# aligirayhanozbay/poisson_CNN

Measured on AMD Instinct MI355X. Metric: grids/sec (fwd+bwd) at 1024^2, higher is better.
Workload: dtype f32; 1 GPU; c4: Homogeneous_Poisson_NN_Legacy(hpnn.json) full train step (fwd+bwd+loss+Adam), 8 x 1024x1024 Dirichlet grids per GPU; global_batch=8, parallelism=dp1, math=fp32, ranks_seen=1

## Files before the change

poisson_cnn_amd/csrc/conv_small.hip:

```cpp
#include "pcnn_internal.h"
#include "conv_epilogue.h"

int pcnn_conv_small_fwd(pcnn_handle h, const pcnn_conv_desc* d, const float* x, const float* w, const float* bias, const float* bn_scale,
                        const float* bn_shift, const float* residual, float* y, float* act_out);
int pcnn_conv_small_wgrad(pcnn_handle h, const pcnn_conv_desc* d, const float* x, const float* dz, float* dw, void* workspace, size_t workspace_bytes);
bool pcnn_conv_fwd_takes_narrow_route(pcnn_handle h, const pcnn_conv_desc* d);
bool pcnn_conv_small_fwd_eligible(const pcnn_conv_desc* d);
bool pcnn_conv_small_wgrad_eligible(const pcnn_conv_desc* d);
size_t pcnn_conv_small_wgrad_workspace(const pcnn_conv_desc* d);

namespace {

constexpr int STH = 8, STW = 32;
__host__ __device__ constexpr int lds_stride(int CI) { return CI == 16 ? 20 : CI; }

struct SmallParams {
  const float* x; const float* wp; const float* bias; const float* bn_scale; const float* bn_shift; const float* res; float* y; float* act_out;
  unsigned* absmax;
  int N, H, W, Cin, ldx, Ho, Wo, Cout, ldy, pt, pl, pad_mode; float pad_value; int act; float alpha;
  int ld_res, ld_act, tiles_x, tiles_y, vec_in, vec_out;
  const float* gact = nullptr; float* y2 = nullptr; float* bpart = nullptr;
  int ld_gact = 0, ld_y2 = 0, gmode = 0; float galpha = 1.f;
};

__device__ __forceinline__ int pad_index_sel(int i, int n, int mode) {
  const int refl = mode == PCNN_PAD_SYMMETRIC ? (i < 0 ? -i - 1 : 2 * n - 1 - i) : (i < 0 ? -i : 2 * n - 2 - i);
  const int rc = min(max(refl, 0), n - 1);
  return (unsigned)i < (unsigned)n ? i : (mode == PCNN_PAD_CONSTANT ? -1 : rc);
}

template <int K, int CI, int CIS = lds_stride(CI)>
__device__ __forceinline__ void stage_tile(float* __restrict__ lds, const float* __restrict__ xin, int H, int W, int Cin, int ldx, int y0, int x0, int pt, int pl,
                                           int pad_mode, float pad_value, int vec) {
  constexpr int TR = STH + K - 1, TC = STW + K - 1, Q = CI / 4;
  for (int u = threadIdx.x; u < TR * TC * Q; u += blockDim.x) {
    const int q = u % Q, pix = u / Q, r = pix / TC, c = pix - r * TC;
    const int sy = pcnn_pad_index(y0 + r - pt, H, pad_mode), sx = pcnn_pad_index(x0 + c - pl, W, pad_mode);
    f32x4 v;
    if (sy < 0 || sx < 0) {
      v = (f32x4){pad_value, pad_value, pad_value, pad_value};
    } else {
      const float* src = xin + ((int64_t)sy * W + sx) * ldx + 4 * q;
      if (vec && 4 * q + 3 < Cin) v = *reinterpret_cast<const f32x4*>(src);
      else {
#pragma unroll
        for (int j = 0; j < 4; ++j) v[j] = 4 * q + j < Cin ? src[j] : 0.f;
      }
    }
#pragma unroll
    for (int j = 0; j < 4; ++j)
      if (4 * q + j >= Cin) v[j] = 0.f;
    *reinterpret_cast<f32x4*>(lds + pix * CIS + 4 * q) = v;
  }
}

template <int K, int CI, int CIS = lds_stride(CI)>
__device__ __forceinline__ void stage_tile_batched(float* __restrict__ lds, const float* __restrict__ xin, int H, int W, int ldx, int y0, int x0, int pt, int pl,
                                                   int pad_mode, float pad_value) {
  constexpr int TR = STH + K - 1, TC = STW + K - 1, Q = CI / 4, TOTAL = TR * TC * Q, NX = (TOTAL + 255) / 256;
  f32x4 v[NX];
  unsigned okm = 0;
#pragma unroll
  for (int i = 0; i < NX; ++i) {
    const int u = threadIdx.x + i * 256, q = u % Q, pix = u / Q, r = pix / TC, c = pix - r * TC;
    const int sy = pad_index_sel(y0 + r - pt, H, pad_mode), sx = pad_index_sel(x0 + c - pl, W, pad_mode);
    const bool ok = u < TOTAL && sy >= 0 && sx >= 0;
    const int64_t idx = ok ? ((int64_t)sy * W + sx) * ldx + 4 * q : 0;
    v[i] = *reinterpret_cast<const f32x4*>(xin + idx);
    okm |= ok ? (1u << i) : 0u;
  }
  const f32x4 padv = {pad_value, pad_value, pad_value, pad_value};
#pragma unroll
  for (int i = 0; i < NX; ++i) {
    const int u = threadIdx.x + i * 256;
    if (u < TOTAL) *reinterpret_cast<f32x4*>(lds + (u / Q) * CIS + 4 * (u % Q)) = ((okm >> i) & 1u) ? v[i] : padv;
  }
}

template <int K, int CI, int CO, bool POST = false>
__global__ __launch_bounds__(256, (CI * CO <= 64 ? 8 : 4)) void conv_small_fwd_kernel(SmallParams p) {
  constexpr int TC = STW + K - 1, CIS = lds_stride(CI);
  extern __shared__ __attribute__((aligned(16))) float lds[];
  int tile = blockIdx.x;
  const int tx = tile % p.tiles_x; tile /= p.tiles_x;
  const int ty = tile % p.tiles_y;
  const int n = tile / p.tiles_y;
  const int y0 = ty * STH, x0 = tx * STW;
  if (p.vec_in && (p.Cin & 3) == 0) stage_tile_batched<K, CI>(lds, p.x + (int64_t)n * p.H * p.W * p.ldx, p.H, p.W, p.ldx, y0, x0, p.pt, p.pl, p.pad_mode, p.pad_value);
  else stage_tile<K, CI>(lds, p.x + (int64_t)n * p.H * p.W * p.ldx, p.H, p.W, p.Cin, p.ldx, y0, x0, p.pt, p.pl, p.pad_mode, p.pad_value, p.vec_in);
  __syncthreads();
  const int r = threadIdx.x >> 5, c = threadIdx.x & 31;
  float acc[CO];
#pragma unroll
  for (int o = 0; o < CO; ++o) acc[o] = 0.f;
  const float* wp = p.wp;
#pragma unroll 1
  for (int i = 0; i < K; ++i)
#pragma unroll
    for (int j = 0; j < K; ++j) {
      const float* px = lds + ((r + i) * TC + (c + j)) * CIS;
      float xv[CI];
#pragma unroll
      for (int q = 0; q < CI / 4; ++q) {
        const f32x4 v = *reinterpret_cast<const f32x4*>(px + 4 * q);
        xv[4 * q] = v[0]; xv[4 * q + 1] = v[1]; xv[4 * q + 2] = v[2]; xv[4 * q + 3] = v[3];
      }
#pragma unroll
      for (int ci = 0; ci < CI; ++ci)
#pragma unroll
        for (int o = 0; o < CO; ++o) acc[o] = fmaf(xv[ci], wp[((i * K + j) * CI + ci) * CO + o], acc[o]);
    }
  const int oy = y0 + r, ox = x0 + c;
  float ymax = 0.f;
  if constexpr (POST) {
    float bs[CO];
#pragma unroll
    for (int o = 0; o < CO; ++o) bs[o] = 0.f;
    if (oy < p.Ho && ox < p.Wo) {
      const int64_t pix = ((int64_t)n * p.Ho + oy) * p.Wo + ox;
      f32x4 rr[CO / 4], gg[CO / 4];
#pragma unroll
      for (int q = 0; q < CO / 4; ++q) {
        const int cq = 4 * q < p.Cout ? 4 * q : 0;
        gg[q] = *reinterpret_cast<const f32x4*>(p.gact + pix * p.ld_gact + cq);
        if (p.res) rr[q] = *reinterpret_cast<const f32x4*>(p.res + pix * p.ld_res + cq);
      }
#pragma unroll
      for (int q = 0; q < CO / 4; ++q) {
        if (4 * q < p.Cout) {
          f32x4 v = {acc[4 * q], acc[4 * q + 1], acc[4 * q + 2], acc[4 * q + 3]};
          if (p.res) {
#pragma unroll
            for (int j = 0; j < 4; ++j) v[j] += rr[q][j];
          }
          if (p.y2) *reinterpret_cast<f32x4*>(p.y2 + pix * p.ld_y2 + 4 * q) = v;
#pragma unroll
          for (int j = 0; j < 4; ++j) {
            const float gq = gg[q][j];
            v[j] *= p.gmode == PCNN_ACT_TANH ? 1.f - gq * gq : (gq > 0.f ? 1.f : p.galpha);
            bs[4 * q + j] = v[j];
            ymax = fmaxf(ymax, fabsf(v[j]));
          }
          *reinterpret_cast<f32x4*>(p.y + pix * p.ldy + 4 * q) = v;
        }
      }
    }
    if (p.bpart) {
      __syncthreads();
#pragma unroll
      for (int o = 0; o < CO; ++o) {
        float v = bs[o];
#pragma unroll
        for (int m = 32; m > 0; m >>= 1) v += __shfl_xor(v, m);
        if ((threadIdx.x & 63) == 0) lds[(threadIdx.x >> 6) * CO + o] = v;
      }
      __syncthreads();
      if (threadIdx.x < CO) p.bpart[(int64_t)blockIdx.x * CO + threadIdx.x] = ((lds[threadIdx.x] + lds[CO + threadIdx.x]) + lds[2 * CO + threadIdx.x]) + lds[3 * CO + threadIdx.x];
    }
    conv_epilogue_absmax(p.absmax, ymax);
    return;
  }
  if (oy < p.Ho && ox < p.Wo) {
    const int64_t pix = ((int64_t)n * p.Ho + oy) * p.Wo + ox;
    float out[CO];
#pragma unroll
    for (int o = 0; o < CO; ++o) {
      float v = 0.f;
      if (o < p.Cout) {
        v = pcnn_act(acc[o] + (p.bias ? p.bias[o] : 0.f), p.act, p.alpha);
        if (p.act_out && !p.vec_out) p.act_out[pix * p.ld_act + o] = v;
      }
      out[o] = v;
    }
    if (p.vec_out) {
      f32x4 rr[CO / 4];
      if (p.res) {
#pragma unroll
        for (int q = 0; q < CO / 4; ++q) rr[q] = *reinterpret_cast<const f32x4*>(p.res + pix * p.ld_res + (4 * q < p.Cout ? 4 * q : 0));
      }
      if (p.act_out) {
#pragma unroll
        for (int q = 0; q < CO / 4; ++q)
          if (4 * q < p.Cout) *reinterpret_cast<f32x4*>(p.act_out + pix * p.ld_act + 4 * q) = (f32x4){out[4 * q], out[4 * q + 1], out[4 * q + 2], out[4 * q + 3]};
      }
#pragma unroll
      for (int q = 0; q < CO / 4; ++q) {
        if (4 * q < p.Cout) {
          f32x4 v = {out[4 * q], out[4 * q + 1], out[4 * q + 2], out[4 * q + 3]};
          if (p.bn_scale) {
#pragma unroll
            for (int j = 0; j < 4; ++j) v[j] = v[j] * p.bn_scale[4 * q + j] + p.bn_shift[4 * q + j];
          }
          if (p.res) {
#pragma unroll
            for (int j = 0; j < 4; ++j) v[j] += rr[q][j];
          }
          *reinterpret_cast<f32x4*>(p.y + pix * p.ldy + 4 * q) = v;
#pragma unroll
          for (int j = 0; j < 4; ++j) ymax = fmaxf(ymax, fabsf(v[j]));
        }
      }
    } else {
#pragma unroll
      for (int o = 0; o < CO; ++o) {
        if (o < p.Cout) {
          float v = out[o];
          if (p.bn_scale) v = v * p.bn_scale[o] + p.bn_shift[o];
          if (p.res) v += p.res[pix * p.ld_res + o];
          p.y[pix * p.ldy + o] = v;
          ymax = fmaxf(ymax, fabsf(v));
        }
      }
    }
  }
  conv_epilogue_absmax(p.absmax, ymax);
}

__global__ void pack_small_kernel(const float* __restrict__ w, float* __restrict__ wp, int taps, int Cin, int Cout, int CI, int CO) {
  const int total = taps * CI * CO;
  for (int i = blockIdx.x * blockDim.x + threadIdx.x; i < total; i += gridDim.x * blockDim.x) {
    const int o = i % CO; int r = i / CO; const int ci = r % CI; const int t = r / CI;
    wp[i] = (ci < Cin && o < Cout) ? w[((int64_t)t * Cin + ci) * Cout + o] : 0.f;
  }
}

template <int K, int CI, int CO>
void launch_small_fwd(pcnn_handle h, const SmallParams& p, int64_t nblk) {
  constexpr size_t lds = (size_t)(STH + K - 1) * (STW + K - 1) * lds_stride(CI) * sizeof(float);
  static_assert(lds >= 4 * 16 * sizeof(float), "the POST epilogue reduces 4 waves x CO sums through the tile's LDS");
  if (p.gact) hipLaunchKernelGGL((conv_small_fwd_kernel<K, CI, CO, true>), dim3((unsigned)nblk), dim3(256), lds, h->stream, p);
  else hipLaunchKernelGGL((conv_small_fwd_kernel<K, CI, CO, false>), dim3((unsigned)nblk), dim3(256), lds, h->stream, p);
}

template <int K, int CI>
bool dispatch_co(pcnn_handle h, const SmallParams& p, int64_t nblk, int CO) {
  switch (CO) {
    case 4: launch_small_fwd<K, CI, 4>(h, p, nblk); return true;
    case 8: launch_small_fwd<K, CI, 8>(h, p, nblk); return true;
    case 12: launch_small_fwd<K, CI, 12>(h, p, nblk); return true;
    case 16: launch_small_fwd<K, CI, 16>(h, p, nblk); return true;
  }
  return false;
}
template <int K>
bool dispatch_ci(pcnn_handle h, const SmallParams& p, int64_t nblk, int CI, int CO) {
  switch (CI) {
    case 4: return dispatch_co<K, 4>(h, p, nblk, CO);
    case 8: return dispatch_co<K, 8>(h, p, nblk, CO);
    case 12: return dispatch_co<K, 12>(h, p, nblk, CO);
    case 16: return dispatch_co<K, 16>(h, p, nblk, CO);
  }
  return false;
}

struct SmallWgradParams {
  const float* x; const float* dz; float* part;
  int N, H, W, Cin, ldx, Ho, Wo, Cout, lddz, pt, pl, pad_mode; float pad_value;
  int tiles_x, tiles_y, ntiles, S, vec_in, vec_dz;
};

template <int K, int CI, int CO>
__global__ __launch_bounds__(64 * K) void conv_small_wgrad_kernel(SmallWgradParams p) {
  constexpr int TR = STH + K - 1, TC = STW + K - 1, CIS = CI, COS = CO;
  constexpr int NT = 64 * K, QX = CI / 4, QZ = CO / 4, NX = (TR * TC * QX + NT - 1) / NT, NZ = (STH * STW * QZ + NT - 1) / NT;
  extern __shared__ __attribute__((aligned(16))) float lds[];
  float* xs = lds;
  float* zs = lds + TR * TC * CIS + 16;
  const int tid = threadIdx.x, lane = tid & 63, ch = lane & 15, kk = lane >> 4;
  const int wave = __builtin_amdgcn_readfirstlane(tid >> 6);
  const int split = blockIdx.x;
  constexpr int GP = CI <= 4 ? 4 : (CI <= 8 ? 2 : 1), CPT = 16 / GP, NM = (K + GP - 1) / GP;
  const int js = ch / CPT, cc = ch % CPT;
  f32x4 acc[NM];
#pragma unroll
  for (int g = 0; g < NM; ++g) acc[g] = (f32x4){0.f, 0.f, 0.f, 0.f};
  const bool b_ok = ch < CO;
  f32x4 xr[NX], zr[NZ];
  unsigned xok = ~0u, zok = ~0u;
  const bool fast = p.vec_in && p.vec_dz && (p.Cin & 3) == 0 && (p.Cout & 3) == 0;
  const f32x4 padv = {p.pad_value, p.pad_value, p.pad_value, p.pad_value}, zero4 = {0.f, 0.f, 0.f, 0.f};
  auto fetch = [&](int tile) {
    int tt = tile;
    const int tx = tt % p.tiles_x; tt /= p.tiles_x;
    const int ty = tt % p.tiles_y;
    const int n = tt / p.tiles_y;
    const int y0 = ty * STH, x0 = tx * STW;
    const float* xin = p.x + (int64_t)n * p.H * p.W * p.ldx;
    const float* zin = p.dz + (int64_t)n * p.Ho * p.Wo * p.lddz;
    if (fast) {
#pragma unroll
      for (int i = 0; i < NX; ++i) {
        const int u = tid + i * NT, q = u % QX, pix = u / QX, r = pix / TC, c = pix - r * TC;
        const int sy = pad_index_sel(y0 + r - p.pt, p.H, p.pad_mode), sx = pad_index_sel(x0 + c - p.pl, p.W, p.pad_mode);
        const bool ok = u < TR * TC * QX && sy >= 0 && sx >= 0;
        xr[i] = *reinterpret_cast<const f32x4*>(xin + (ok ? ((int64_t)sy * p.W + sx) * p.ldx + 4 * q : 0));
        xok = ok ? (xok | (1u << i)) : (xok & ~(1u << i));
      }
#pragma unroll
      for (int i = 0; i < NZ; ++i) {
        const int u = tid + i * NT, q = u % QZ, pix = u / QZ, r = pix / STW, c = pix - r * STW;
        const bool ok = u < STH * STW * QZ && y0 + r < p.Ho && x0 + c < p.Wo;
        zr[i] = *reinterpret_cast<const f32x4*>(zin + (ok ? ((int64_t)(y0 + r) * p.Wo + x0 + c) * p.lddz + 4 * q : 0));
        zok = ok ? (zok | (1u << i)) : (zok & ~(1u << i));
      }
      return;
    }
#pragma unroll
    for (int i = 0; i < NX; ++i) {
      const int u = tid + i * NT, q = u % QX, pix = u / QX, r = pix / TC, c = pix - r * TC;
      f32x4 v = {0.f, 0.f, 0.f, 0.f};
      if (u < TR * TC * QX) {
        const int sy = pcnn_pad_index(y0 + r - p.pt, p.H, p.pad_mode), sx = pcnn_pad_index(x0 + c - p.pl, p.W, p.pad_mode);
        if (sy < 0 || sx < 0) v = (f32x4){p.pad_value, p.pad_value, p.pad_value, p.pad_value};
        else {
          const float* src = xin + ((int64_t)sy * p.W + sx) * p.ldx + 4 * q;
          if (p.vec_in && 4 * q + 3 < p.Cin) v = *reinterpret_cast<const f32x4*>(src);
          else {
#pragma unroll
            for (int j = 0; j < 4; ++j) v[j] = 4 * q + j < p.Cin ? src[j] : 0.f;
          }
        }
#pragma unroll
        for (int j = 0; j < 4; ++j)
          if (4 * q + j >= p.Cin) v[j] = 0.f;
      }
      xr[i] = v;
    }
#pragma unroll
    for (int i = 0; i < NZ; ++i) {
      const int u = tid + i * NT, q = u % QZ, pix = u / QZ, r = pix / STW, c = pix - r * STW;
      f32x4 v = {0.f, 0.f, 0.f, 0.f};
      if (u < STH * STW * QZ && y0 + r < p.Ho && x0 + c < p.Wo) {
        const float* src = zin + ((int64_t)(y0 + r) * p.Wo + x0 + c) * p.lddz + 4 * q;
        if (p.vec_dz && 4 * q + 3 < p.Cout) v = *reinterpret_cast<const f32x4*>(src);
        else {
#pragma unroll
          for (int j = 0; j < 4; ++j) v[j] = 4 * q + j < p.Cout ? src[j] : 0.f;
        }
      }
      zr[i] = v;
    }
  };
  int tile = split;
  if (tile < p.ntiles) fetch(tile);
  for (; tile < p.ntiles; tile += p.S) {
    __syncthreads();
#pragma unroll
    for (int i = 0; i < NX; ++i) {
      const int u = tid + i * NT;
      if (u < TR * TC * QX) *reinterpret_cast<f32x4*>(xs + (u / QX) * CIS + 4 * (u % QX)) = ((xok >> i) & 1u) ? xr[i] : padv;
    }
#pragma unroll
    for (int i = 0; i < NZ; ++i) {
      const int u = tid + i * NT;
      if (u < STH * STW * QZ) *reinterpret_cast<f32x4*>(zs + (u / QZ) * COS + 4 * (u % QZ)) = ((zok >> i) & 1u) ? zr[i] : zero4;
    }
    __syncthreads();
    if (tile + p.S < p.ntiles) fetch(tile + p.S);
#pragma unroll 1
    for (int r = 0; r < STH; ++r) {
      const float* zrow = zs + (r * STW + kk) * COS + ch;
      const float* xrow = xs + ((r + wave) * TC + kk + js) * CIS + cc;
#pragma unroll
      for (int c0 = 0; c0 < STW; c0 += 4) {
        float bv = zrow[c0 * COS];
        bv = b_ok ? bv : 0.f;
#pragma unroll
        for (int g = 0; g < NM; ++g) {
          float av = xrow[(c0 + g * GP) * CIS];
          av = (cc < CI && g * GP + js < K) ? av : 0.f;
          acc[g] = __builtin_amdgcn_mfma_f32_16x16x4f32(av, bv, acc[g], 0, 0, 0);
        }
      }
    }
  }
#pragma unroll
  for (int g = 0; g < NM; ++g)
#pragma unroll
    for (int r = 0; r < 4; ++r) {
      const int row = 4 * kk + r, j = g * GP + row / CPT, ci = row % CPT;
      if (j < K && ci < p.Cin && ch < p.Cout) p.part[(((int64_t)split * K * K + wave * K + j) * p.Cin + ci) * p.Cout + ch] = acc[g][r];
    }
}

__global__ __launch_bounds__(256) void small_wgrad_reduce_kernel(const float* __restrict__ part, float* __restrict__ dw, int nel, int S) {
  __shared__ float red[16][16];
  const int el = threadIdx.x & 15, q = threadIdx.x >> 4, e = blockIdx.x * 16 + el;
  float s = 0.f;
  if (e < nel)
    for (int k = q; k < S; k += 16) s += part[(int64_t)k * nel + e];
  red[q][el] = s;
  __syncthreads();
  if (q == 0 && e < nel) {
    float t = 0.f;
#pragma unroll
    for (int i = 0; i < 16; ++i) t += red[i][el];
    dw[e] = t;
  }
}

size_t wgrad_lds_bytes(int K, int CI, int CO) { return ((size_t)(STH + K - 1) * (STW + K - 1) * CI + 16 + (size_t)STH * STW * CO + 16) * sizeof(float); }

int wgrad_splits(const pcnn_conv_desc* d) {
  const int64_t ntiles = (int64_t)d->N * pcnn_cdiv(d->Ho, STH) * pcnn_cdiv(d->Wo, STW);
  const int per_cu = (int)std::min<size_t>(8, (160u << 10) / wgrad_lds_bytes(d->kh, (d->Cin + 3) & ~3, (d->Cout + 3) & ~3));
  return (int)std::min<int64_t>(ntiles, 256 * per_cu);
}

template <int K, int CI, int CO>
void launch_small_wgrad(pcnn_handle h, const SmallWgradParams& p) {
  hipLaunchKernelGGL((conv_small_wgrad_kernel<K, CI, CO>), dim3((unsigned)p.S), dim3(64 * K), wgrad_lds_bytes(K, CI, CO), h->stream, p);
}
template <int K, int CI>
bool wgrad_dispatch_co(pcnn_handle h, const SmallWgradParams& p, int CO) {
  switch (CO) {
    case 4: launch_small_wgrad<K, CI, 4>(h, p); return true;
    case 8: launch_small_wgrad<K, CI, 8>(h, p); return true;
    case 12: launch_small_wgrad<K, CI, 12>(h, p); return true;
    case 16: launch_small_wgrad<K, CI, 16>(h, p); return true;
  }
  return false;
}
template <int K>
bool wgrad_dispatch_ci(pcnn_handle h, const SmallWgradParams& p, int CI, int CO) {
  switch (CI) {
    case 4: return wgrad_dispatch_co<K, 4>(h, p, CO);
    case 8: return wgrad_dispatch_co<K, 8>(h, p, CO);
    case 12: return wgrad_dispatch_co<K, 12>(h, p, CO);
    case 16: return wgrad_dispatch_co<K, 16>(h, p, CO);
  }
  return false;
}


struct StageParams {
  const float* x; const float* w0; const float* w1; const float* w2; const float* b0; const float* b1; const float* b2;
  float* o0; float* a1; float* o1; float* y;
  int N, H, W, tiles_x, tiles_y; float slope;
};

typedef const float __attribute__((address_space(4))) * const_weights;

template <int C>
__device__ __forceinline__ void stage_conv3(const float* __restrict__ src, int pitch, const float* wg, float (&acc)[C]) {
  const const_weights w = (const_weights)wg;
#pragma unroll 1
  for (int i = 0; i < 3; ++i)
#pragma unroll
    for (int j = 0; j < 3; ++j) {
      const float* px = src + (i * pitch + j) * C;
      float xv[C];
#pragma unroll
      for (int q = 0; q < C / 4; ++q) {
        const f32x4 v = *reinterpret_cast<const f32x4*>(px + 4 * q);
        xv[4 * q] = v[0]; xv[4 * q + 1] = v[1]; xv[4 * q + 2] = v[2]; xv[4 * q + 3] = v[3];
      }
#pragma unroll
      for (int ci = 0; ci < C; ++ci)
#pragma unroll
        for (int o = 0; o < C; ++o) acc[o] = fmaf(xv[ci], w[((i * 3 + j) * C + ci) * C + o], acc[o]);
    }
}

template <int C, int TH>
__global__ __launch_bounds__(256) void resnet3_stage_kernel(StageParams p) {
  constexpr int XR = TH + 6, XC = STW + 6, R0 = TH + 4, C0 = STW + 4, R1 = TH + 2, C1 = STW + 2, Q = C / 4;
  constexpr int TOTAL = XR * XC * Q, NX = (TOTAL + 255) / 256;
  extern __shared__ __attribute__((aligned(16))) float lds[];
  float* const X = lds;
  float* const O0 = lds + XR * XC * C;
  int tile = blockIdx.x;
  const int tx = tile % p.tiles_x; tile /= p.tiles_x;
  const int ty = tile % p.tiles_y;
  const int n = tile / p.tiles_y;
  const int y0 = ty * TH, x0 = tx * STW;
  const int64_t img = (int64_t)n * p.H * p.W * C;
  {
    const float* xin = p.x + img;
    f32x4 v[NX];
    unsigned okm = 0;
#pragma unroll
    for (int i = 0; i < NX; ++i) {
      const int u = threadIdx.x + i * 256, q = u % Q, pix = u / Q, r = pix / XC, c = pix - r * XC;
      const int sy = y0 + r - 3, sx = x0 + c - 3;
      const bool ok = u < TOTAL && (unsigned)sy < (unsigned)p.H && (unsigned)sx < (unsigned)p.W;
      v[i] = *reinterpret_cast<const f32x4*>(xin + (ok ? ((int64_t)sy * p.W + sx) * C + 4 * q : 0));
      okm |= ok ? (1u << i) : 0u;
    }
    const f32x4 z4 = {0.f, 0.f, 0.f, 0.f};
#pragma unroll
    for (int i = 0; i < NX; ++i) {
      const int u = threadIdx.x + i * 256;
      if (u < TOTAL) *reinterpret_cast<f32x4*>(X + (u / Q) * C + 4 * (u % Q)) = ((okm >> i) & 1u) ? v[i] : z4;
    }
  }
  __syncthreads();
  auto bias_act = [&](float (&acc)[C], const float* bg) {
    const const_weights b = (const_weights)bg;
#pragma unroll
    for (int o = 0; o < C; ++o) { const float t = acc[o] + (bg ? b[o] : 0.f); acc[o] = t > 0.f ? t : p.slope * t; }
  };
  auto store_px = [&](float* dst, int gy, int gx, const float (&val)[C]) {
    float* d = dst + img + ((int64_t)gy * p.W + gx) * C;
#pragma unroll
    for (int q = 0; q < Q; ++q) *reinterpret_cast<f32x4*>(d + 4 * q) = (f32x4){val[4 * q], val[4 * q + 1], val[4 * q + 2], val[4 * q + 3]};
  };
#pragma unroll 1
  for (int idx = threadIdx.x; idx < R0 * C0; idx += 256) {
    const int r = idx / C0, c = idx - r * C0, gy = y0 - 2 + r, gx = x0 - 2 + c;
    float acc[C];
#pragma unroll
    for (int o = 0; o < C; ++o) acc[o] = 0.f;
    stage_conv3<C>(X + (r * XC + c) * C, XC, p.w0, acc);
    bias_act(acc, p.b0);
    const bool inside = (unsigned)gy < (unsigned)p.H && (unsigned)gx < (unsigned)p.W;
#pragma unroll
    for (int q = 0; q < Q; ++q)
      *reinterpret_cast<f32x4*>(O0 + idx * C + 4 * q) = inside ? (f32x4){acc[4 * q], acc[4 * q + 1], acc[4 * q + 2], acc[4 * q + 3]} : (f32x4){0.f, 0.f, 0.f, 0.f};
    if (p.o0 && inside && r >= 2 && r < TH + 2 && c >= 2 && c < STW + 2) store_px(p.o0, gy, gx, acc);
  }
  __syncthreads();
#pragma unroll 1
  for (int idx = threadIdx.x; idx < R1 * C1; idx += 256) {
    const int r = idx / C1, c = idx - r * C1, gy = y0 - 1 + r, gx = x0 - 1 + c;
    float acc[C];
#pragma unroll
    for (int o = 0; o < C; ++o) acc[o] = 0.f;
    stage_conv3<C>(O0 + (r * C0 + c) * C, C0, p.w1, acc);
    bias_act(acc, p.b1);
    const bool inside = (unsigned)gy < (unsigned)p.H && (unsigned)gx < (unsigned)p.W;
    const bool own = inside && r >= 1 && r < TH + 1 && c >= 1 && c < STW + 1;
    if (p.a1 && own) store_px(p.a1, gy, gx, acc);
    float* xs = X + ((r + 2) * XC + (c + 2)) * C;
    float s[C];
#pragma unroll
    for (int q = 0; q < Q; ++q) {
      const f32x4 xv = *reinterpret_cast<const f32x4*>(xs + 4 * q);
#pragma unroll
      for (int j = 0; j < 4; ++j) s[4 * q + j] = inside ? xv[j] + acc[4 * q + j] : 0.f;
      *reinterpret_cast<f32x4*>(xs + 4 * q) = (f32x4){s[4 * q], s[4 * q + 1], s[4 * q + 2], s[4 * q + 3]};
    }
    if (p.o1 && own) store_px(p.o1, gy, gx, s);
  }
  __syncthreads();
#pragma unroll 1
  for (int idx = threadIdx.x; idx < TH * STW; idx += 256) {
    const int r = idx >> 5, c = idx & 31, gy = y0 + r, gx = x0 + c;
    float acc[C];
#pragma unroll
    for (int o = 0; o < C; ++o) acc[o] = 0.f;
    stage_conv3<C>(X + ((r + 2) * XC + (c + 2)) * C, XC, p.w2, acc);
    bias_act(acc, p.b2);
    if (gy < p.H && gx < p.W) store_px(p.y, gy, gx, acc);
  }
}

template <int C, int TH>
void launch_stage(pcnn_handle h, StageParams p) {
  constexpr size_t lds = ((size_t)(TH + 6) * (STW + 6) + (size_t)(TH + 4) * (STW + 4)) * C * sizeof(float);
  (void)hipFuncSetAttribute(reinterpret_cast<const void*>(resnet3_stage_kernel<C, TH>), hipFuncAttributeMaxDynamicSharedMemorySize, (int)lds);
  p.tiles_x = pcnn_cdiv(p.W, STW); p.tiles_y = pcnn_cdiv(p.H, TH);
  hipLaunchKernelGGL((resnet3_stage_kernel<C, TH>), dim3((unsigned)(p.N * p.tiles_x * p.tiles_y)), dim3(256), lds, h->stream, p);
}

__global__ __launch_bounds__(256) void small_post_bias_kernel(const float* __restrict__ bpart, int64_t nblk, int CO, float* __restrict__ dbias) {
  __shared__ float red[256];
  const int ch = blockIdx.x, t = threadIdx.x;
  float a = 0.f;
  for (int64_t b = t; b < nblk; b += 256) a += bpart[b * CO + ch];
  red[t] = a;
  __syncthreads();
  for (int st = 128; st > 0; st >>= 1) { if (t < st) red[t] += red[t + st]; __syncthreads(); }
  if (t == 0) dbias[ch] = red[0];
}

}

static int pad4(int c) { return (c + 3) & ~3; }

bool pcnn_conv_small_fwd_eligible(const pcnn_conv_desc* d) {
  if (d->kh != d->kw || (d->kh != 3 && d->kh != 5) || d->Cin > 16 || d->Cout > 16) return false;
  if (d->kh == 5 && pad4(d->Cin) * pad4(d->Cout) > 16 * 16) return false;
  return true;
}

bool pcnn_conv_small_wgrad_eligible(const pcnn_conv_desc* d) {
  return d->kh == d->kw && (d->kh == 3 || d->kh == 5) && d->Cin <= 16 && d->Cout <= 16;
}

size_t pcnn_conv_small_wgrad_workspace(const pcnn_conv_desc* d) {
  return pcnn_conv_small_wgrad_eligible(d) ? (size_t)wgrad_splits(d) * d->kh * d->kw * d->Cin * d->Cout * sizeof(float) : 0;
}

static int small_fwd_impl(pcnn_handle h, const pcnn_conv_desc* d, const float* x, const float* w, const float* bias, const float* bn_scale,
                          const float* bn_shift, const float* residual, float* y, float* act_out, const pcnn_post_desc* post);

int pcnn_conv_small_fwd(pcnn_handle h, const pcnn_conv_desc* d, const float* x, const float* w, const float* bias, const float* bn_scale,
                        const float* bn_shift, const float* residual, float* y, float* act_out) {
  return small_fwd_impl(h, d, x, w, bias, bn_scale, bn_shift, residual, y, act_out, nullptr);
}

static bool quads_ok(const void* q, int ld) { return q == nullptr || ((reinterpret_cast<uintptr_t>(q) & 15) == 0 && ld % 4 == 0); }
extern "C" int pcnn_conv2d_dgrad_post_eligible(pcnn_handle h, const pcnn_conv_desc* dg, const float* dz, const float* residual, const float* dx, const pcnn_post_desc* post) {
  if (!h || !dg || !post || !post->act_out) return 0;
  if (dg->pad_mode != PCNN_PAD_CONSTANT || dg->act != PCNN_ACT_LINEAR || dg->N < 1) return 0;
  if (!pcnn_conv_small_fwd_eligible(dg) || !pcnn_conv_fwd_takes_narrow_route(h, dg)) return 0;
  if (dg->Cout % 4 != 0) return 0;
  if (post->act != PCNN_ACT_LINEAR && post->act != PCNN_ACT_RELU && post->act != PCNN_ACT_LEAKY_RELU && post->act != PCNN_ACT_TANH) return 0;
  return (quads_ok(dx, dg->ldy) && quads_ok(residual, dg->ld_res) && quads_ok(post->act_out, post->ld_act_out) && quads_ok(post->raw_out, post->ld_raw) && dz) ? 1 : 0;
}
extern "C" int pcnn_conv2d_dgrad_post(pcnn_handle h, const pcnn_conv_desc* dg, const float* dz, const float* w_flipped, const float* residual, float* dx,
                                      const pcnn_post_desc* post) {
  PCNN_REQUIRE(h, h && dg && dz && w_flipped && dx && post, "pcnn_conv2d_dgrad_post: null argument");
  PCNN_REQUIRE(h, pcnn_conv2d_dgrad_post_eligible(h, dg, dz, residual, dx, post), "pcnn_conv2d_dgrad_post: not eligible (ask pcnn_conv2d_dgrad_post_eligible first)");
  return small_fwd_impl(h, dg, dz, w_flipped, nullptr, nullptr, nullptr, residual, dx, nullptr, post);
}

static int small_fwd_impl(pcnn_handle h, const pcnn_conv_desc* d, const float* x, const float* w, const float* bias, const float* bn_scale,
                          const float* bn_shift, const float* residual, float* y, float* act_out, const pcnn_post_desc* post) {
  const int CI = pad4(d->Cin), CO = pad4(d->Cout), taps = d->kh * d->kw;
  const size_t need = (size_t)taps * CI * CO * sizeof(float);
  if (h->scratch_bytes < need) {
    if (h->scratch) { pcnn_release(h, h->scratch); h->scratch = nullptr; h->scratch_bytes = 0; }
    const size_t cap = 4u << 20;
    if (hipMalloc(&h->scratch, cap) != hipSuccess) PCNN_FAIL(h, "pcnn_conv2d_fwd: cannot allocate %zu B of filter scratch", cap);
    h->scratch_bytes = cap;
  }
  float* wp = static_cast<float*>(h->scratch);
  hipLaunchKernelGGL(pack_small_kernel, dim3(pcnn_cdiv(taps * CI * CO, 256)), dim3(256), 0, h->stream, w, wp, taps, d->Cin, d->Cout, CI, CO);
  SmallParams p;
  p.x = x; p.wp = wp; p.bias = bias; p.bn_scale = bn_scale; p.bn_shift = bn_shift; p.res = residual; p.y = y; p.act_out = act_out;
  p.absmax = reinterpret_cast<unsigned*>(h->y_absmax);
  p.N = d->N; p.H = d->H; p.W = d->W; p.Cin = d->Cin; p.ldx = d->ldx; p.Ho = d->Ho; p.Wo = d->Wo; p.Cout = d->Cout; p.ldy = d->ldy;
  p.pt = d->pad_top; p.pl = d->pad_left; p.pad_mode = d->pad_mode; p.pad_value = d->pad_value; p.act = d->act; p.alpha = d->act_alpha;
  p.ld_res = d->ld_res; p.ld_act = d->ld_act_out;
  p.tiles_x = pcnn_cdiv(d->Wo, STW); p.tiles_y = pcnn_cdiv(d->Ho, STH);
  p.vec_in = (d->ldx % 4 == 0) && ((reinterpret_cast<uintptr_t>(x) & 15) == 0);
  p.vec_out = conv_epilogue_vec_ok(d->Cout, y, d->ldy, residual, d->ld_res, act_out, d->ld_act_out);
  const int64_t nblk = (int64_t)d->N * p.tiles_x * p.tiles_y;
  PCNN_REQUIRE(h, nblk < (1ll << 31), "pcnn_conv2d_fwd: grid too large");
  if (post) {
    p.gact = post->act_out; p.ld_gact = post->ld_act_out; p.y2 = post->raw_out; p.ld_y2 = post->ld_raw; p.gmode = post->act;
    p.galpha = post->act == PCNN_ACT_LINEAR ? 1.f : (post->act == PCNN_ACT_RELU ? 0.f : post->act_alpha);
    if (post->dbias) {
      const size_t need = (size_t)nblk * CO * sizeof(float);
      if (h->aux_ws_bytes < need) {
        if (h->aux_ws) { pcnn_release(h, h->aux_ws); h->aux_ws = nullptr; h->aux_ws_bytes = 0; }
        if (hipMalloc(&h->aux_ws, need) != hipSuccess) PCNN_FAIL(h, "pcnn_conv2d_dgrad_post: cannot allocate %zu B of scratch", need);
        h->aux_ws_bytes = need;
      }
      p.bpart = static_cast<float*>(h->aux_ws);
    }
  }
  const bool ok = d->kh == 3 ? dispatch_ci<3>(h, p, nblk, CI, CO) : dispatch_ci<5>(h, p, nblk, CI, CO);
  PCNN_REQUIRE(h, ok, "pcnn_conv2d_fwd(small): no kernel for %d->%d", d->Cin, d->Cout);
  PCNN_CHECK_LAUNCH(h, "pcnn_conv2d_fwd(small)");
  if (post && post->dbias) {
    hipLaunchKernelGGL(small_post_bias_kernel, dim3((unsigned)d->Cout), dim3(256), 0, h->stream, p.bpart, nblk, CO, post->dbias);
    PCNN_CHECK_LAUNCH(h, "pcnn_conv2d_dgrad_post(bias)");
  }
  return 0;
}

int pcnn_conv_small_wgrad(pcnn_handle h, const pcnn_conv_desc* d, const float* x, const float* dz, float* dw, void* workspace, size_t workspace_bytes) {
  PCNN_REQUIRE(h, workspace_bytes >= pcnn_conv_small_wgrad_workspace(d), "pcnn_conv2d_wgrad(small): workspace too small");
  const int CI = pad4(d->Cin), CO = pad4(d->Cout);
  SmallWgradParams p;
  p.x = x; p.dz = dz; p.part = static_cast<float*>(workspace);
  p.N = d->N; p.H = d->H; p.W = d->W; p.Cin = d->Cin; p.ldx = d->ldx; p.Ho = d->Ho; p.Wo = d->Wo; p.Cout = d->Cout; p.lddz = d->ldy;
  p.pt = d->pad_top; p.pl = d->pad_left; p.pad_mode = d->pad_mode; p.pad_value = d->pad_value;
  p.tiles_x = pcnn_cdiv(d->Wo, STW); p.tiles_y = pcnn_cdiv(d->Ho, STH); p.ntiles = d->N * p.tiles_x * p.tiles_y; p.S = wgrad_splits(d);
  p.vec_in = (d->ldx % 4 == 0) && ((reinterpret_cast<uintptr_t>(x) & 15) == 0);
  p.vec_dz = (d->ldy % 4 == 0) && ((reinterpret_cast<uintptr_t>(dz) & 15) == 0);
  const bool ok = d->kh == 3 ? wgrad_dispatch_ci<3>(h, p, CI, CO) : wgrad_dispatch_ci<5>(h, p, CI, CO);
  PCNN_REQUIRE(h, ok, "pcnn_conv2d_wgrad(small): no kernel for %d->%d", d->Cin, d->Cout);
  PCNN_CHECK_LAUNCH(h, "pcnn_conv2d_wgrad(small)");
  const int nel = d->kh * d->kw * d->Cin * d->Cout;
  hipLaunchKernelGGL(small_wgrad_reduce_kernel, dim3(pcnn_cdiv(nel, 16)), dim3(256), 0, h->stream, p.part, dw, nel, p.S);
  PCNN_CHECK_LAUNCH(h, "pcnn_conv2d_wgrad(small reduce)");
  return 0;
}

extern "C" int pcnn_resnet3_fwd_eligible(pcnn_handle h, int C, int act) {
  return (h && (C == 4 || C == 8) && (act == PCNN_ACT_LINEAR || act == PCNN_ACT_RELU || act == PCNN_ACT_LEAKY_RELU)) ? 1 : 0;
}

extern "C" int pcnn_resnet3_fwd(pcnn_handle h, int N, int H, int W, int C, int act, float act_alpha, const float* x, const float* w0, const float* b0,
                                const float* w1, const float* b1, const float* w2, const float* b2, float* o0, float* a1, float* o1, float* y) {
  PCNN_REQUIRE(h, h && x && w0 && w1 && w2 && y, "pcnn_resnet3_fwd: null argument");
  PCNN_REQUIRE(h, pcnn_resnet3_fwd_eligible(h, C, act), "pcnn_resnet3_fwd: %d channels / activation %d are not eligible (ask pcnn_resnet3_fwd_eligible first)", C, act);
  PCNN_REQUIRE(h, N >= 1 && H >= 1 && W >= 1, "pcnn_resnet3_fwd: bad shape");
  for (const void* q : {(const void*)x, (const void*)o0, (const void*)a1, (const void*)o1, (const void*)y})
    PCNN_REQUIRE(h, (reinterpret_cast<uintptr_t>(q) & 15) == 0, "pcnn_resnet3_fwd: tensors must be 16-byte aligned");
  PCNN_REQUIRE(h, (int64_t)N * pcnn_cdiv(W, STW) * pcnn_cdiv(H, 8) < (1ll << 31), "pcnn_resnet3_fwd: grid too large");
  StageParams p;
  p.x = x; p.w0 = w0; p.w1 = w1; p.w2 = w2; p.b0 = b0; p.b1 = b1; p.b2 = b2; p.o0 = o0; p.a1 = a1; p.o1 = o1; p.y = y;
  p.N = N; p.H = H; p.W = W; p.tiles_x = 0; p.tiles_y = 0;
  p.slope = act == PCNN_ACT_LINEAR ? 1.f : (act == PCNN_ACT_RELU ? 0.f : act_alpha);
  const bool tall = H > 8;
  if (C == 4) { if (tall) launch_stage<4, 16>(h, p); else launch_stage<4, 8>(h, p); }
  else { if (tall) launch_stage<8, 16>(h, p); else launch_stage<8, 8>(h, p); }
  PCNN_CHECK_LAUNCH(h, "pcnn_resnet3_fwd");
  return 0;
}
```

Baseline: 43.50 grids/s.

## Pack more kernel taps per MFMA tile in small-channel conv weight-gradient kernel

```diff
diff --git a/poisson_cnn_amd/csrc/conv_small.hip b/poisson_cnn_amd/csrc/conv_small.hip
--- a/poisson_cnn_amd/csrc/conv_small.hip
+++ b/poisson_cnn_amd/csrc/conv_small.hip
@@ -259,22 +259,81 @@
   int tiles_x, tiles_y, ntiles, S, vec_in, vec_dz;
 };
 
+struct WgradPlan {
+  int NB, BS;
+  int NAX, AS;
+  int NAY;
+  int NW, NMT;
+  int WPS;
+  int SX, TXA;
+  bool full;
+};
+__host__ __device__ constexpr int cdiv_c(int a, int b) { return (a + b - 1) / b; }
+__host__ __device__ constexpr WgradPlan wgrad_plan(int K, int CI, int CO) {
+  WgradPlan P{};
+  P.NB = 16 / CO < K ? 16 / CO : K;
+  if (P.NB == 1) { P.BS = 0; P.NAX = K; P.AS = 1; }
+  else if (P.NB == 2) { P.BS = (K + 1) / 2; P.NAX = P.BS; P.AS = 1; }
+  else { P.BS = 1; P.AS = P.NB; P.NAX = cdiv_c(K, P.NB); }
+  const int RA = P.NAX * CI;
+  P.full = cdiv_c(K * RA, 16) < K * cdiv_c(RA, 16);
+  P.NAY = P.full ? K : 1;
+  P.NW = P.full ? 4 : K;
+  P.NMT = P.full ? cdiv_c(K * RA, 16) : cdiv_c(RA, 16);
+  P.WPS = !P.full ? 1 : P.NMT <= 1 ? 8 : P.NMT <= 2 ? 6 : P.NMT <= 7 ? 4 : 2;
+  P.SX = (P.NB - 1) * P.BS;
+  P.TXA = (P.NAX - 1) * P.AS;
+  return P;
+}
+__host__ __device__ constexpr int wgrad_block_tap(int K, int CI, int CO, int ix, int b) {
+  const WgradPlan P = wgrad_plan(K, CI, CO);
+  const int t = ix * P.AS + b * P.BS;
+  if (t >= K) return -1;
+  for (int i = 0; i <= ix; ++i)
+    for (int c = 0; c < P.NB; ++c)
+      if ((i < ix || c < b) && i * P.AS + c * P.BS == t) return -1;
+  return t;
+}
+__host__ __device__ constexpr bool wgrad_plan_ok(int K, int CI, int CO) {
+  const WgradPlan P = wgrad_plan(K, CI, CO);
+  for (int t = 0; t < K; ++t) {
+    int n = 0;
+    for (int ix = 0; ix < P.NAX; ++ix)
+      for (int b = 0; b < P.NB; ++b) n += wgrad_block_tap(K, CI, CO, ix, b) == t;
+    if (n != 1) return false;
+  }
+  for (int ix = 0; ix < P.NAX; ++ix) if (ix * P.AS > P.TXA) return false;
+  for (int b = 0; b < P.NB; ++b) if (b * P.BS > P.SX) return false;
+  if (P.NB * CO > 16 || P.NMT * 16 < P.NAY * P.NAX * CI || P.NMT * 16 >= P.NAY * P.NAX * CI + 16) return false;
+  if (P.full && (P.NW != 4 || STH % P.NW != 0)) return false;
+  return true;
+}
+
 template <int K, int CI, int CO>
-__global__ __launch_bounds__(64 * K) void conv_small_wgrad_kernel(SmallWgradParams p) {
-  constexpr int TR = STH + K - 1, TC = STW + K - 1, CIS = CI, COS = CO;
-  constexpr int NT = 64 * K, QX = CI / 4, QZ = CO / 4, NX = (TR * TC * QX + NT - 1) / NT, NZ = (STH * STW * QZ + NT - 1) / NT;
+__global__ __launch_bounds__(64 * wgrad_plan(K, CI, CO).NW, wgrad_plan(K, CI, CO).WPS) void conv_small_wgrad_kernel(SmallWgradParams p) {
+  constexpr WgradPlan P = wgrad_plan(K, CI, CO);
+  static_assert(wgrad_plan_ok(K, CI, CO), "packing plan: a tap is produced twice or not at all, or a shift leaves the staged halo");
+  constexpr int TR = STH + K - 1, TC = STW + P.TXA, TCZ = STW + P.SX, CIS = CI, COS = CO;
+  constexpr int NT = 64 * P.NW, QX = CI / 4, QZ = CO / 4, TOTX = TR * TC * QX, TOTZ = STH * TCZ * QZ, NX = (TOTX + NT - 1) / NT, NZ = (TOTZ + NT - 1) / NT;
+  constexpr int NMT = P.NMT, NA = P.NAY * P.NAX;
+  static_assert(!P.full || TR * TC * CIS >= NT * 4, "the cross-wave sum goes through the input tile's LDS");
   extern __shared__ __attribute__((aligned(16))) float lds[];
   float* xs = lds;
   float* zs = lds + TR * TC * CIS + 16;
   const int tid = threadIdx.x, lane = tid & 63, ch = lane & 15, kk = lane >> 4;
   const int wave = __builtin_amdgcn_readfirstlane(tid >> 6);
   const int split = blockIdx.x;
-  constexpr int GP = CI <= 4 ? 4 : (CI <= 8 ? 2 : 1), CPT = 16 / GP, NM = (K + GP - 1) / GP;
-  const int js = ch / CPT, cc = ch % CPT;
-  f32x4 acc[NM];
-#pragma unroll
-  for (int g = 0; g < NM; ++g) acc[g] = (f32x4){0.f, 0.f, 0.f, 0.f};
-  const bool b_ok = ch < CO;
+  int offA[NMT];
+#pragma unroll
+  for (int g = 0; g < NMT; ++g) {
+    const int m = 16 * g + ch, a = min(m / CI, NA - 1), iy = a / P.NAX, ix = a - iy * P.NAX;
+    offA[g] = (iy * TC + ix * P.AS) * CIS + (m - a * CI);
+  }
+  const int bg = min(ch / CO, P.NB - 1), offB = (P.SX - bg * P.BS) * COS + (ch - bg * CO);
+  const int wy = P.full ? 0 : wave, r0 = P.full ? wave * (STH / P.NW) : 0, r1 = P.full ? r0 + STH / P.NW : STH;
+  f32x4 acc[NMT];
+#pragma unroll
+  for (int g = 0; g < NMT; ++g) acc[g] = (f32x4){0.f, 0.f, 0.f, 0.f};
   f32x4 xr[NX], zr[NZ];
   unsigned xok = ~0u, zok = ~0u;
   const bool fast = p.vec_in && p.vec_dz && (p.Cin & 3) == 0 && (p.Cout & 3) == 0;
@@ -292,15 +351,15 @@
       for (int i = 0; i < NX; ++i) {
         const int u = tid + i * NT, q = u % QX, pix = u / QX, r = pix / TC, c = pix - r * TC;
         const int sy = pad_index_sel(y0 + r - p.pt, p.H, p.pad_mode), sx = pad_index_sel(x0 + c - p.pl, p.W, p.pad_mode);
-        const bool ok = u < TR * TC * QX && sy >= 0 && sx >= 0;
+        const bool ok = u < TOTX && sy >= 0 && sx >= 0;
         xr[i] = *reinterpret_cast<const f32x4*>(xin + (ok ? ((int64_t)sy * p.W + sx) * p.ldx + 4 * q : 0));
         xok = ok ? (xok | (1u << i)) : (xok & ~(1u << i));
       }
 #pragma unroll
       for (int i = 0; i < NZ; ++i) {
-        const int u = tid + i * NT, q = u % QZ, pix = u / QZ, r = pix / STW, c = pix - r * STW;
-        const bool ok = u < STH * STW * QZ && y0 + r < p.Ho && x0 + c < p.Wo;
-        zr[i] = *reinterpret_cast<const f32x4*>(zin + (ok ? ((int64_t)(y0 + r) * p.Wo + x0 + c) * p.lddz + 4 * q : 0));
+        const int u = tid + i * NT, q = u % QZ, pix = u / QZ, r = pix / TCZ, c = pix - r * TCZ, gx = x0 - P.SX + c;
+        const bool ok = u < TOTZ && y0 + r < p.Ho && gx < p.Wo && (P.SX == 0 || gx >= 0);
+        zr[i] = *reinterpret_cast<const f32x4*>(zin + (ok ? ((int64_t)(y0 + r) * p.Wo + x0 + c - P.SX) * p.lddz + 4 * q : 0));
         zok = ok ? (zok | (1u << i)) : (zok & ~(1u << i));
       }
       return;
@@ -309,7 +368,7 @@
     for (int i = 0; i < NX; ++i) {
       const int u = tid + i * NT, q = u % QX, pix = u / QX, r = pix / TC, c = pix - r * TC;
       f32x4 v = {0.f, 0.f, 0.f, 0.f};
-      if (u < TR * TC * QX) {
+      if (u < TOTX) {
         const int sy = pcnn_pad_index(y0 + r - p.pt, p.H, p.pad_mode), sx = pcnn_pad_index(x0 + c - p.pl, p.W, p.pad_mode);
         if (sy < 0 || sx < 0) v = (f32x4){p.pad_value, p.pad_value, p.pad_value, p.pad_value};
         else {
@@ -328,10 +387,10 @@
     }
 #pragma unroll
     for (int i = 0; i < NZ; ++i) {
-      const int u = tid + i * NT, q = u % QZ, pix = u / QZ, r = pix / STW, c = pix - r * STW;
+      const int u = tid + i * NT, q = u % QZ, pix = u / QZ, r = pix / TCZ, c = pix - r * TCZ, gx = x0 - P.SX + c;
       f32x4 v = {0.f, 0.f, 0.f, 0.f};
-      if (u < STH * STW * QZ && y0 + r < p.Ho && x0 + c < p.Wo) {
-        const float* src = zin + ((int64_t)(y0 + r) * p.Wo + x0 + c) * p.lddz + 4 * q;
+      if (u < TOTZ && y0 + r < p.Ho && gx < p.Wo && (P.SX == 0 || gx >= 0)) {
+        const float* src = zin + ((int64_t)(y0 + r) * p.Wo + x0 + c - P.SX) * p.lddz + 4 * q;
         if (p.vec_dz && 4 * q + 3 < p.Cout) v = *reinterpret_cast<const f32x4*>(src);
         else {
 #pragma unroll
@@ -348,39 +407,51 @@
 #pragma unroll
     for (int i = 0; i < NX; ++i) {
       const int u = tid + i * NT;
-      if (u < TR * TC * QX) *reinterpret_cast<f32x4*>(xs + (u / QX) * CIS + 4 * (u % QX)) = ((xok >> i) & 1u) ? xr[i] : padv;
+      if (u < TOTX) *reinterpret_cast<f32x4*>(xs + (u / QX) * CIS + 4 * (u % QX)) = ((xok >> i) & 1u) ? xr[i] : padv;
     }
 #pragma unroll
     for (int i = 0; i < NZ; ++i) {
       const int u = tid + i * NT;
-      if (u < STH * STW * QZ) *reinterpret_cast<f32x4*>(zs + (u / QZ) * COS + 4 * (u % QZ)) = ((zok >> i) & 1u) ? zr[i] : zero4;
+      if (u < TOTZ) *reinterpret_cast<f32x4*>(zs + (u / QZ) * COS + 4 * (u % QZ)) = ((zok >> i) & 1u) ? zr[i] : zero4;
     }
     __syncthreads();
     if (tile + p.S < p.ntiles) fetch(tile + p.S);
 #pragma unroll 1
-    for (int r = 0; r < STH; ++r) {
-      const float* zrow = zs + (r * STW + kk) * COS + ch;
-      const float* xrow = xs + ((r + wave) * TC + kk + js) * CIS + cc;
+    for (int r = r0; r < r1; ++r) {
+      const float* zrow = zs + (r * TCZ + kk) * COS + offB;
+      const float* xrow = xs + ((r + wy) * TC + kk) * CIS;
 #pragma unroll
       for (int c0 = 0; c0 < STW; c0 += 4) {
-        float bv = zrow[c0 * COS];
-        bv = b_ok ? bv : 0.f;
-#pragma unroll
-        for (int g = 0; g < NM; ++g) {
-          float av = xrow[(c0 + g * GP) * CIS];
-          av = (cc < CI && g * GP + js < K) ? av : 0.f;
-          acc[g] = __builtin_amdgcn_mfma_f32_16x16x4f32(av, bv, acc[g], 0, 0, 0);
-        }
-      }
-    }
-  }
-#pragma unroll
-  for (int g = 0; g < NM; ++g)
-#pragma unroll
-    for (int r = 0; r < 4; ++r) {
-      const int row = 4 * kk + r, j = g * GP + row / CPT, ci = row % CPT;
-      if (j < K && ci < p.Cin && ch < p.Cout) p.part[(((int64_t)split * K * K + wave * K + j) * p.Cin + ci) * p.Cout + ch] = acc[g][r];
-    }
+        const float bv = zrow[c0 * COS];
+#pragma unroll
+        for (int g = 0; g < NMT; ++g) acc[g] = __builtin_amdgcn_mfma_f32_16x16x4f32(xrow[c0 * CIS + offA[g]], bv, acc[g], 0, 0, 0);
+      }
+    }
+  }
+  auto put = [&](int g, int r, int lq, float v) {
+    const int m = 16 * g + 4 * lq + r, a = m / CI, ci = m - a * CI, iy = a / P.NAX, ix = a - iy * P.NAX, b = ch / CO, co = ch - b * CO;
+    if (a >= NA || b >= P.NB) return;
+    const int dx = wgrad_block_tap(K, CI, CO, ix, b), dy = P.full ? iy : wave;
+    if (dx >= 0 && ci < p.Cin && co < p.Cout) p.part[(((int64_t)split * K * K + dy * K + dx) * p.Cin + ci) * p.Cout + co] = v;
+  };
+  if constexpr (P.full) {
+#pragma unroll
+    for (int g = 0; g < NMT; ++g) {
+      __syncthreads();
+#pragma unroll
+      for (int r = 0; r < 4; ++r) xs[(wave * 4 + r) * 64 + lane] = acc[g][r];
+      __syncthreads();
+      float s = xs[wave * 64 + lane];
+#pragma unroll
+      for (int w = 1; w < 4; ++w) s += xs[(w * 4 + wave) * 64 + lane];
+      put(g, wave, kk, s);
+    }
+  } else {
+#pragma unroll
+    for (int g = 0; g < NMT; ++g)
+#pragma unroll
+      for (int r = 0; r < 4; ++r) put(g, r, kk, acc[g][r]);
+  }
 }
 
 __global__ __launch_bounds__(256) void small_wgrad_reduce_kernel(const float* __restrict__ part, float* __restrict__ dw, int nel, int S) {
@@ -399,17 +470,23 @@
   }
 }
 
-size_t wgrad_lds_bytes(int K, int CI, int CO) { return ((size_t)(STH + K - 1) * (STW + K - 1) * CI + 16 + (size_t)STH * STW * CO + 16) * sizeof(float); }
+size_t wgrad_lds_bytes(int K, int CI, int CO) {
+  const WgradPlan P = wgrad_plan(K, CI, CO);
+  return ((size_t)(STH + K - 1) * (STW + P.TXA) * CI + 16 + (size_t)STH * (STW + P.SX) * CO + 16) * sizeof(float);
+}
+int wgrad_tiles_x(const pcnn_conv_desc* d) { return pcnn_cdiv(d->Wo + wgrad_plan(d->kh, (d->Cin + 3) & ~3, (d->Cout + 3) & ~3).SX, STW); }
 
 int wgrad_splits(const pcnn_conv_desc* d) {
-  const int64_t ntiles = (int64_t)d->N * pcnn_cdiv(d->Ho, STH) * pcnn_cdiv(d->Wo, STW);
-  const int per_cu = (int)std::min<size_t>(8, (160u << 10) / wgrad_lds_bytes(d->kh, (d->Cin + 3) & ~3, (d->Cout + 3) & ~3));
+  const int64_t ntiles = (int64_t)d->N * pcnn_cdiv(d->Ho, STH) * wgrad_tiles_x(d);
+  const WgradPlan P = wgrad_plan(d->kh, (d->Cin + 3) & ~3, (d->Cout + 3) & ~3);
+  int per_cu = (int)std::min<size_t>(8, (160u << 10) / wgrad_lds_bytes(d->kh, (d->Cin + 3) & ~3, (d->Cout + 3) & ~3));
+  if (P.full) per_cu = std::min(per_cu, P.WPS * 4 / P.NW);
   return (int)std::min<int64_t>(ntiles, 256 * per_cu);
 }
 
 template <int K, int CI, int CO>
 void launch_small_wgrad(pcnn_handle h, const SmallWgradParams& p) {
-  hipLaunchKernelGGL((conv_small_wgrad_kernel<K, CI, CO>), dim3((unsigned)p.S), dim3(64 * K), wgrad_lds_bytes(K, CI, CO), h->stream, p);
+  hipLaunchKernelGGL((conv_small_wgrad_kernel<K, CI, CO>), dim3((unsigned)p.S), dim3(64 * wgrad_plan(K, CI, CO).NW), wgrad_lds_bytes(K, CI, CO), h->stream, p);
 }
 template <int K, int CI>
 bool wgrad_dispatch_co(pcnn_handle h, const SmallWgradParams& p, int CO) {
@@ -669,7 +746,7 @@
   p.x = x; p.dz = dz; p.part = static_cast<float*>(workspace);
   p.N = d->N; p.H = d->H; p.W = d->W; p.Cin = d->Cin; p.ldx = d->ldx; p.Ho = d->Ho; p.Wo = d->Wo; p.Cout = d->Cout; p.lddz = d->ldy;
   p.pt = d->pad_top; p.pl = d->pad_left; p.pad_mode = d->pad_mode; p.pad_value = d->pad_value;
-  p.tiles_x = pcnn_cdiv(d->Wo, STW); p.tiles_y = pcnn_cdiv(d->Ho, STH); p.ntiles = d->N * p.tiles_x * p.tiles_y; p.S = wgrad_splits(d);
+  p.tiles_x = wgrad_tiles_x(d); p.tiles_y = pcnn_cdiv(d->Ho, STH); p.ntiles = d->N * p.tiles_x * p.tiles_y; p.S = wgrad_splits(d);
   p.vec_in = (d->ldx % 4 == 0) && ((reinterpret_cast<uintptr_t>(x) & 15) == 0);
   p.vec_dz = (d->ldy % 4 == 0) && ((reinterpret_cast<uintptr_t>(dz) & 15) == 0);
   const bool ok = d->kh == 3 ? wgrad_dispatch_ci<3>(h, p, CI, CO) : wgrad_dispatch_ci<5>(h, p, CI, CO);
```

After: 43.79 grids/s (median of 6 runs). No clear change (+0.7%).
